# saiakarsh193/GenVox

Hardware: NVIDIA B200
Metric: Tacotron2 train mel-frames/s (higher is better)
Workload: dtype bf16

## Files before the change

genvox_b200/_native.py:

```python
import ctypes as C
import os

from . import build as _build

_P = C.c_void_p


class GvxDims(C.Structure):
    _fields_ = [("n_mels", C.c_int32), ("enc_dim", C.c_int32), ("att_rnn_dim", C.c_int32), ("dec_rnn_dim", C.c_int32),
                ("prenet_dim", C.c_int32), ("att_dim", C.c_int32), ("loc_filters", C.c_int32), ("loc_kernel", C.c_int32),
                ("p_att_dropout", C.c_float), ("p_dec_dropout", C.c_float), ("precision", C.c_int32)]


PARAM_FIELDS = [
    ("prenet_w0", "prenet.layers.0.linear_layer.weight"),
    ("prenet_w1", "prenet.layers.1.linear_layer.weight"),
    ("att_w_ih", "attention_rnn.weight_ih"),
    ("att_w_hh", "attention_rnn.weight_hh"),
    ("att_b_ih", "attention_rnn.bias_ih"),
    ("att_b_hh", "attention_rnn.bias_hh"),
    ("query_w", "attention_layer.query_layer.linear_layer.weight"),
    ("memory_w", "attention_layer.memory_layer.linear_layer.weight"),
    ("v_w", "attention_layer.v.linear_layer.weight"),
    ("loc_conv_w", "attention_layer.location_layer.location_conv.conv.weight"),
# ... 39 lines not shown
    "gvx_dec_packed_bytes": (C.c_size_t, [C.POINTER(GvxDims)]),
    "gvx_dec_pack_weights": (C.c_int, [C.POINTER(GvxDims), C.POINTER(GvxWeights), _P, _P]),
    "gvx_dec_stash_bytes": (C.c_size_t, [C.POINTER(GvxDims), C.c_int, C.c_int, C.c_int]),
    "gvx_dec_bwd_workspace_bytes": (C.c_size_t, [C.POINTER(GvxDims), C.c_int, C.c_int, C.c_int]),
    "gvx_dec_infer_workspace_bytes": (C.c_size_t, [C.POINTER(GvxDims), C.c_int, C.c_int, C.c_int]),
    "gvx_dec_train_fwd": (C.c_int, [C.POINTER(GvxDims), C.POINTER(GvxWeights), _P, _P, _P, _P, C.c_int, C.c_int, C.c_int,
                                    C.c_uint64, C.c_int, C.c_int, _P, _P, _P, _P, _P]),
    "gvx_dec_train_bwd": (C.c_int, [C.POINTER(GvxDims), C.POINTER(GvxWeights), _P, _P, _P, C.c_int, C.c_int, C.c_int,
                                    C.c_uint64, C.c_int, C.c_int, _P, _P, _P, _P, _P, C.POINTER(GvxGrads), _P, _P]),
    "gvx_dec_infer": (C.c_int, [C.POINTER(GvxDims), C.POINTER(GvxWeights), _P, _P, _P, C.c_int, C.c_int, C.c_int,
                                C.c_float, C.c_int, C.c_uint64, C.c_int, C.c_int, _P, _P, _P, _P, C.POINTER(C.c_int), _P, _P]),
    "gvx_dec_infer_continuous_workspace_bytes": (C.c_size_t, [C.POINTER(GvxDims), C.c_int, C.c_int, C.c_int]),
    "gvx_dec_infer_continuous": (C.c_int, [C.POINTER(GvxDims), C.POINTER(GvxWeights), _P, _P, _P, C.c_int, C.c_int, C.c_int,
                                           C.c_int, _P, C.c_float, C.c_int, C.c_uint64, C.c_int, _P, _P, _P, _P,
                                           C.POINTER(C.c_longlong), _P, _P]),
    "gvx_dec_session_workspace_bytes": (C.c_size_t, [C.POINTER(GvxDims), C.c_int, C.c_int, C.c_int]),
    "gvx_dec_session_init": (C.c_int, [C.POINTER(GvxDims), C.POINTER(GvxSession), _P, _P]),
    "gvx_dec_session_submit": (C.c_int, [C.POINTER(GvxDims), C.POINTER(GvxWeights), _P, C.POINTER(GvxSession), _P, _P, _P,
                                         C.c_int, _P, _P]),
    "gvx_dec_session_step": (C.c_int, [C.POINTER(GvxDims), C.POINTER(GvxWeights), _P, C.POINTER(GvxSession), C.c_int,
                                       _P, _P, _P, _P, _P, C.POINTER(C.c_int), _P, _P]),
    "gvx_test_tc_gemm": (C.c_int, [_P, _P, C.c_int, C.c_int, C.c_int, C.c_int, _P, _P]),
    "gvx_test_nt_gemm": (C.c_int, [_P, _P, C.c_int, C.c_int, C.c_int, C.c_int, _P, _P]),
    "gvx_bench_nt_gemm": (C.c_int, [C.c_int, C.c_int, C.c_int, C.c_int, C.POINTER(C.c_float)]),
    "gvx_test_lstm_chain": (C.c_int, [_P, _P, C.c_int, C.c_int, C.c_int, C.c_float, C.c_uint64, C.c_int, _P, _P, _P, _P, _P, _P]),
    "gvx_debug_timeline": (C.c_int, [_P]),
    "gvx_debug_option": (C.c_int, [C.c_char_p, C.c_int]),
    "gvx_prenet_fwd": (C.c_int, [C.POINTER(GvxDims), C.POINTER(GvxWeights), _P, C.c_int, C.c_int, C.c_uint64, C.c_int,
                                 C.c_int, _P, _P, _P]),
    "gvx_lstm_step": (C.c_int, [C.POINTER(GvxDims), _P, C.c_int, _P, _P, _P, C.c_int, C.c_uint64, C.c_int, C.c_int,
                                C.c_int, _P, _P, _P, _P]),
    "gvx_attention_step": (C.c_int, [C.POINTER(GvxDims), C.POINTER(GvxWeights), _P, _P, _P, _P, _P, C.c_int, C.c_int,
                                     _P, _P, _P, _P, _P, _P]),
}

EXPORTS = sorted(_SIGNATURES)
_lib = None


def library_path():
    return _build.LIB_PATH


def library_is_fresh():
    return _build.is_fresh()


# ... 37 lines not shown
```

genvox_b200/csrc/gvx_bf16_api.cuh:

```cuda
#pragma once
#include <cublas_v2.h>

#include "gvx_attention_c2.cuh"
#include "gvx_bf16.cuh"
#include "gvx_blas.cuh"
#include "gvx_layout.cuh"
#include "gvx_misc.cuh"
#include "gvx_fused_fwd.cuh"
#include "gvx_fused_bwd.cuh"
#include "gvx_nt_gemm.cuh"
#include "gvx_infer_prenet.cuh"
#include "gvx_persist.cuh"

namespace gvx {

typedef __nv_bfloat16 bf16;

inline int round_up(int x, int m) { return (x + m - 1) / m * m; }

struct BfGeom {
    int Kpa, Kpd, Kpq, Kpp, Dp;
    int Ta, Td, Tq, Tp;
    int TaT, TdT, TqT;
    int G4A, G4H;
// ... 884 lines not shown
size_t bwd_total_bf16(const Dims &d, int B, int N, int T) { return BwdBfL(d, B, N, T).total; }
size_t infer_total_bf16(const Dims &d, int B, int N, int steps) { return InferBfL(d, B, N, steps).total; }
size_t stash_seed_off_bf16(const Dims &d, int B, int N, int T) { return StashBfL(d, B, N, T).SEED; }
size_t infer_flags_off_bf16(const Dims &d, int B, int N, int steps) { return InferBfL(d, B, N, steps).FLAGS; }
size_t infer_err_off_bf16(const Dims &d, int B, int N, int steps) { return InferBfL(d, B, N, steps).ERR; }
int check_tc_err_public(int *err_dev, cudaStream_t st, const char *what) { return check_tc_err(err_dev, st, what); }

}

extern "C" int gvx_debug_option(const char *name, int value) {
    if (!strcmp(name, "fused")) gvx::fa_mode() = value;
    else if (!strcmp(name, "persistent")) gvx::pc_mode() = value;
    else { snprintf(gvx::g_err, sizeof(gvx::g_err), "gvx_debug_option: unknown option %s", name); return 1; }
    return 0;
}

extern "C" int gvx_debug_timeline(void *device_buffer) {
    gvx::pc_dbg_buffer() = (long long *)device_buffer;
    return 0;
}

extern "C" int gvx_test_nt_gemm(const float *A, const float *B, int M, int N, int K, int mode, float *C, void *stream) {
    using namespace gvx;
    GVX_CHECK(A && B && C && M > 0 && N > 0 && K > 0 && K % 8 == 0, "bad argument");
    cudaStream_t st = (cudaStream_t)stream;
    bf16 *a = nullptr, *b = nullptr, *at = nullptr, *bt = nullptr;
    int *err = nullptr;
    float *ws = nullptr;
    const size_t ws_floats = (size_t)32 << 20;
    GVX_CUDA(cudaMalloc(&a, (size_t)M * K * 2));
    GVX_CUDA(cudaMalloc(&b, (size_t)N * K * 2));
    GVX_CUDA(cudaMalloc(&err, 64));
    GVX_CUDA(cudaMalloc(&ws, ws_floats * 4));
    GVX_CUDA(cudaMemsetAsync(err, 0, 64, st));
    int rc = 0;
    if (mode == 0) {
        k_to_bf16<<<grid_for((size_t)M * K), 256, 0, st>>>(A, K, (size_t)M, K, a, K);
        k_to_bf16<<<grid_for((size_t)N * K), 256, 0, st>>>(B, K, (size_t)N, K, b, K);
        rc = nt_gemm_bf16(st, M, N, K, a, K, b, K, C, N, err, ws, ws_floats);
    } else {
        GVX_CHECK(M % 8 == 0 && N % 8 == 0, "mode 1 needs M, N multiples of 8");
        k_to_bf16<<<grid_for((size_t)M * K), 256, 0, st>>>(A, M, (size_t)K, M, a, M);
        k_to_bf16<<<grid_for((size_t)N * K), 256, 0, st>>>(B, N, (size_t)K, N, b, N);
        rc = tn_gemm_bf16(st, M, N, K, a, M, b, N, C, N, err, ws, ws_floats);
    }
    if (!rc) rc = check_tc_err(err, st, "nt_gemm");
    else cudaStreamSynchronize(st);
    cudaFree(a); cudaFree(b); cudaFree(at); cudaFree(bt); cudaFree(err); cudaFree(ws);
    return rc;
}

extern "C" int gvx_bench_nt_gemm(int M, int N, int K, int reps, float *ms_out) {
    using namespace gvx;
    bf16 *a = nullptr, *b = nullptr;
    float *c = nullptr, *ws = nullptr;
    int *err = nullptr;
    const size_t ws_floats = (size_t)32 << 20;
    GVX_CUDA(cudaMalloc(&ws, ws_floats * 4));
    GVX_CUDA(cudaMalloc(&a, (size_t)M * K * 2));
    GVX_CUDA(cudaMalloc(&b, (size_t)N * K * 2));
    GVX_CUDA(cudaMalloc(&c, (size_t)M * N * 4));
    GVX_CUDA(cudaMalloc(&err, 64));
    GVX_CUDA(cudaMemset(a, 0, (size_t)M * K * 2));
    GVX_CUDA(cudaMemset(b, 0, (size_t)N * K * 2));
    GVX_CUDA(cudaMemset(err, 0, 64));
    cudaEvent_t e0, e1;
    cudaEventCreate(&e0); cudaEventCreate(&e1);
    int rc = nt_gemm_bf16(0, M, N, K, a, K, b, K, c, N, err, ws, ws_floats);
    cudaEventRecord(e0, 0);
    for (int i = 0; i < reps && !rc; ++i) rc = nt_gemm_bf16(0, M, N, K, a, K, b, K, c, N, err, ws, ws_floats);
    cudaEventRecord(e1, 0);
    cudaEventSynchronize(e1);
    float ms = 0.f;
    cudaEventElapsedTime(&ms, e0, e1);
    *ms_out = ms / (reps > 0 ? reps : 1);
    if (!rc) rc = check_tc_err(err, 0, "nt_gemm bench");
    cudaFree(a); cudaFree(b); cudaFree(c); cudaFree(err); cudaFree(ws);
    cudaEventDestroy(e0); cudaEventDestroy(e1);
    return rc;
}

__global__ void k_bf16_rows_to_f32(const __nv_bfloat16 *__restrict__ x, size_t n, float *__restrict__ y) {
    for (size_t i = (size_t)blockIdx.x * blockDim.x + threadIdx.x; i < n; i += (size_t)gridDim.x * blockDim.x) y[i] = __bfloat162float(x[i]);
}

extern "C" int gvx_test_lstm_chain(const float *w_hh, const float *pre, int B, int T, int H, float p_drop, uint64_t seed,
                                   int training, float *h_out, float *c_out, float *gates_out, const float *dh_ext,
                                   float *dgates_out, void *stream) {
    using namespace gvx;
    GVX_CHECK(w_hh && pre && h_out && c_out && gates_out && B > 0 && T > 0, "bad argument");
    GVX_CHECK(pc_supported(H, B), "persistent chain: unsupported shape (need H % 64 == 0, H/8 <= SM count, B <= 64)");
    cudaStream_t st = (cudaStream_t)stream;
    bf16 *wimg = nullptr, *wimgT = nullptr, *himg = nullptr, *hrm = nullptr, *gimg = nullptr, *dgrm = nullptr;
// ... 44 lines not shown
```

genvox_b200/csrc/gvx_nt_gemm.cuh:

```cuda
#pragma once
#include <cuda.h>
#include <cuda_bf16.h>

#include "gvx_tc.cuh"

namespace gvx {

constexpr int NG_BM = 128, NG_BN = 256, NG_BK = 64;
constexpr int NG_STAGES = 4;
constexpr int NG_STAGE_BYTES = (NG_BM + NG_BN) * NG_BK * 2;
constexpr int NG_THREADS = 192;

struct NgShared {
    uint64_t full[NG_STAGES], empty[NG_STAGES], tfull[2], tempty[2];
    uint32_t tmem_slot;
};
constexpr size_t NG_SMEM = (size_t)NG_STAGES * NG_STAGE_BYTES + sizeof(NgShared) + 1024;

__device__ __forceinline__ void tma_load_2d(void *smem_dst, const CUtensorMap *tm, int c0, int c1, uint64_t *bar) {
    asm volatile("cp.async.bulk.tensor.2d.shared::cluster.global.tile.mbarrier::complete_tx::bytes [%0], [%1, {%2, %3}], [%4];" ::"r"(
                     smem_u32(smem_dst)),
                 "l"(reinterpret_cast<uint64_t>(tm)), "r"(c0), "r"(c1), "r"(smem_u32(bar))
                 : "memory");
}
__device__ __forceinline__ void tmem_ld32(uint32_t taddr, float *v) {
    uint32_t r[32];
    asm volatile(
        "tcgen05.ld.sync.aligned.32x32b.x32.b32 "
        "{%0, %1, %2, %3, %4, %5, %6, %7, %8, %9, %10, %11, %12, %13, %14, %15, %16, %17, %18, %19, %20, %21, %22, %23, %24, %25, %26, "
        "%27, %28, %29, %30, %31}, [%32];"
        : "=r"(r[0]), "=r"(r[1]), "=r"(r[2]), "=r"(r[3]), "=r"(r[4]), "=r"(r[5]), "=r"(r[6]), "=r"(r[7]), "=r"(r[8]), "=r"(r[9]),
          "=r"(r[10]), "=r"(r[11]), "=r"(r[12]), "=r"(r[13]), "=r"(r[14]), "=r"(r[15]), "=r"(r[16]), "=r"(r[17]), "=r"(r[18]),
          "=r"(r[19]), "=r"(r[20]), "=r"(r[21]), "=r"(r[22]), "=r"(r[23]), "=r"(r[24]), "=r"(r[25]), "=r"(r[26]), "=r"(r[27]),
          "=r"(r[28]), "=r"(r[29]), "=r"(r[30]), "=r"(r[31])
        : "r"(taddr));
    asm volatile("tcgen05.wait::ld.sync.aligned;" ::: "memory");
#pragma unroll
    for (int i = 0; i < 32; ++i) v[i] = __uint_as_float(r[i]);
}
__device__ __forceinline__ void mbar_arrive_local(uint64_t *bar) {
    asm volatile("mbarrier.arrive.shared::cta.b64 _, [%0];" ::"r"(smem_u32(bar)) : "memory");
}

struct NgArgs {
    float *C;
    int M, N, K, ldc, tiles_m, tiles_n;
    int splits;
    float *P;
    int *err;
};

template <bool MN>
__global__ void __launch_bounds__(NG_THREADS, 1) k_nt_gemm(const __grid_constant__ CUtensorMap tmA, const __grid_constant__ CUtensorMap tmB,
                                                           const NgArgs a) {
    extern __shared__ uint8_t smem_raw[];
    uint8_t *smem = smem_raw + ((1024u - (smem_u32(smem_raw) & 1023u)) & 1023u);
    NgShared *sh = (NgShared *)(smem + (size_t)NG_STAGES * NG_STAGE_BYTES);
    const int warp = threadIdx.x >> 5, lane = threadIdx.x & 31;
    const int ntiles = a.tiles_m * a.tiles_n * a.splits, nkb_all = (a.K + NG_BK - 1) / NG_BK;
    auto item_of = [&](int item, int &tm, int &tn, int &kb0, int &kb1, int &sp) {
        const int t = item / a.splits;
        sp = item - t * a.splits;
        tm = t / a.tiles_n;
        tn = t - tm * a.tiles_n;
        kb0 = (int)((long long)nkb_all * sp / a.splits);
        kb1 = (int)((long long)nkb_all * (sp + 1) / a.splits);
    };

    if (threadIdx.x == 0) {
        for (int s = 0; s < NG_STAGES; ++s) { mbar_init(sh->full + s, 1); mbar_init(sh->empty + s, 1); }
        for (int k = 0; k < 2; ++k) { mbar_init(sh->tfull + k, 1); mbar_init(sh->tempty + k, 4); }
        asm volatile("fence.mbarrier_init.release.cluster;" ::: "memory");
        asm volatile("fence.proxy.async.shared::cta;" ::: "memory");
    }
    if (warp == 0) {
        asm volatile("tcgen05.alloc.cta_group::1.sync.aligned.shared::cta.b32 [%0], %1;" ::"r"(smem_u32(&sh->tmem_slot)), "n"(512) : "memory");
        asm volatile("tcgen05.relinquish_alloc_permit.cta_group::1.sync.aligned;" ::: "memory");
    }
    tc_fence_before();
    __syncthreads();
    tc_fence_after();
    const uint32_t tmem_base = sh->tmem_slot;

    if (warp == 0) {
        if (elect_one()) {
            int s = 0;
            uint32_t ph = 0;
            for (int tile = blockIdx.x; tile < ntiles; tile += gridDim.x) {
                int tm, tn, kb0, kb1, sp;
                item_of(tile, tm, tn, kb0, kb1, sp);
                for (int kb = kb0; kb < kb1; ++kb) {
                    if (!mbar_wait(sh->empty + s, ph ^ 1u, a.err, 71)) return;
                    uint8_t *dst = smem + (size_t)s * NG_STAGE_BYTES;
                    mbar_expect_tx(sh->full + s, NG_STAGE_BYTES);
                    if (MN) {
#pragma unroll
                        for (int q = 0; q < NG_BM / 64; ++q) tma_load_2d(dst + q * 8192, &tmA, tm * NG_BM + 64 * q, kb * NG_BK, sh->full + s);
#pragma unroll
                        for (int q = 0; q < NG_BN / 64; ++q)
                            tma_load_2d(dst + NG_BM * NG_BK * 2 + q * 8192, &tmB, tn * NG_BN + 64 * q, kb * NG_BK, sh->full + s);
                    } else {
                        tma_load_2d(dst, &tmA, kb * NG_BK, tm * NG_BM, sh->full + s);
                        tma_load_2d(dst + NG_BM * NG_BK * 2, &tmB, kb * NG_BK, tn * NG_BN, sh->full + s);
                    }
                    if (++s == NG_STAGES) { s = 0; ph ^= 1u; }
                }
            }
        }
    } else if (warp == 1) {
        if (elect_one()) {
            constexpr uint32_t idesc = umma_idesc_bf16(NG_BM, NG_BN) | (MN ? (1u << 15) | (1u << 16) : 0u);
            constexpr int kstep = MN ? (2048 >> 4) : 2;
            const uint64_t ad0 = MN ? umma_desc_sw128_mn(smem_u32(smem)) : umma_desc_sw128(smem_u32(smem));
            int s = 0, it = 0;
            uint32_t ph = 0;
            for (int tile = blockIdx.x; tile < ntiles; tile += gridDim.x, ++it) {
                const int acc = it & 1;
                if (!mbar_wait(sh->tempty + acc, (uint32_t)((it >> 1) & 1) ^ 1u, a.err, 72)) return;
                tc_fence_after();
                const uint32_t tacc = tmem_base + (uint32_t)(acc * NG_BN);
                int tm, tn, kb0, kb1, sp;
                item_of(tile, tm, tn, kb0, kb1, sp);
                for (int kb = kb0; kb < kb1; ++kb) {
                    if (!mbar_wait(sh->full + s, ph, a.err, 73)) return;
                    tc_fence_after();
                    const uint64_t ad = ad0 + (uint64_t)(s * (NG_STAGE_BYTES >> 4)), bd = ad + (uint64_t)((NG_BM * NG_BK * 2) >> 4);
#pragma unroll
                    for (int j = 0; j < NG_BK / 16; ++j) umma_bf16(tacc, ad + kstep * j, bd + kstep * j, idesc, (kb > kb0 || j > 0) ? 1u : 0u);
                    umma_commit(sh->empty + s);
                    if (++s == NG_STAGES) { s = 0; ph ^= 1u; }
                }
                umma_commit(sh->tfull + acc);
            }
        }
    } else {
        const int q = warp & 3;
        int it = 0;
        for (int tile = blockIdx.x; tile < ntiles; tile += gridDim.x, ++it) {
            const int acc = it & 1;
            int tm, tn, kb0, kb1, sp;
            item_of(tile, tm, tn, kb0, kb1, sp);
            if (!mbar_wait(sh->tfull + acc, (uint32_t)((it >> 1) & 1), a.err, 74)) return;
            tc_fence_after();
            const int m = tm * NG_BM + 32 * q + lane;
            const int ldc = a.splits > 1 ? a.N : a.ldc;
            float *crow = (a.splits > 1 ? a.P + (size_t)sp * a.M * a.N : a.C) + (size_t)m * ldc + tn * NG_BN;
#pragma unroll 1
            for (int c0 = 0; c0 < NG_BN; c0 += 32) {
                float v[32];
                tmem_ld32(tmem_base + ((uint32_t)(32 * q) << 16) + (uint32_t)(acc * NG_BN + c0), v);
                if (m < a.M) {
                    const int nrem = a.N - (tn * NG_BN + c0);
                    if (nrem >= 32 && (ldc & 3) == 0) {
#pragma unroll
                        for (int i = 0; i < 32; i += 4) *reinterpret_cast<float4 *>(crow + c0 + i) = make_float4(v[i], v[i + 1], v[i + 2], v[i + 3]);
                    } else {
#pragma unroll
                        for (int i = 0; i < 32; ++i)
                            if (i < nrem) crow[c0 + i] = v[i];
                    }
                }
            }
            tc_fence_before();
            __syncwarp();
            if (lane == 0) mbar_arrive_local(sh->tempty + acc);
        }
    }
    __syncthreads();
    if (warp == 0) {
        asm volatile("tcgen05.dealloc.cta_group::1.sync.aligned.b32 %0, %1;" ::"r"(tmem_base), "n"(512) : "memory");
    }
}

typedef CUresult (*PFN_encodeTiled)(CUtensorMap *, CUtensorMapDataType, cuuint32_t, void *, const cuuint64_t *, const cuuint64_t *,
                                    const cuuint32_t *, const cuuint32_t *, CUtensorMapInterleave, CUtensorMapSwizzle,
                                    CUtensorMapL2promotion, CUtensorMapFloatOOBfill);
inline PFN_encodeTiled ng_encode_fn() {
    static PFN_encodeTiled fn = nullptr;
    if (!fn) {
        void *p = nullptr;
        cudaDriverEntryPointQueryResult q;
        if (cudaGetDriverEntryPoint("cuTensorMapEncodeTiled", &p, cudaEnableDefault, &q) == cudaSuccess && q == cudaDriverEntryPointSuccess)
            fn = (PFN_encodeTiled)p;
    }
    return fn;
}
inline int ng_tensor_map_mn(CUtensorMap *tm, const __nv_bfloat16 *base, int K, int MNsize, int ld) {
    PFN_encodeTiled fn = ng_encode_fn();
    GVX_CHECK(fn != nullptr, "cuTensorMapEncodeTiled is not available from this driver");
    GVX_CHECK(((uintptr_t)base & 15) == 0 && ld % 8 == 0, "tn_gemm: operands must be 16-byte aligned with a row stride that is a multiple of 8");
    const cuuint64_t dims[2] = {(cuuint64_t)MNsize, (cuuint64_t)K};
    const cuuint64_t strides[1] = {(cuuint64_t)ld * 2};
    const cuuint32_t box[2] = {64u, (cuuint32_t)NG_BK};
// ... 12 lines not shown
    GVX_CHECK(((uintptr_t)base & 15) == 0 && ld % 8 == 0, "nt_gemm: operands must be 16-byte aligned with a row stride that is a multiple of 8");
    const cuuint64_t dims[2] = {(cuuint64_t)K, (cuuint64_t)rows};
    const cuuint64_t strides[1] = {(cuuint64_t)ld * 2};
    const cuuint32_t box[2] = {(cuuint32_t)NG_BK, (cuuint32_t)box_rows};
    const cuuint32_t estr[2] = {1, 1};
    const CUresult r = fn(tm, CU_TENSOR_MAP_DATA_TYPE_BFLOAT16, 2, (void *)base, dims, strides, box, estr, CU_TENSOR_MAP_INTERLEAVE_NONE,
                          CU_TENSOR_MAP_SWIZZLE_128B, CU_TENSOR_MAP_L2_PROMOTION_L2_256B, CU_TENSOR_MAP_FLOAT_OOB_FILL_NONE);
    if (r != CUDA_SUCCESS) {
        snprintf(g_err, sizeof(g_err), "cuTensorMapEncodeTiled failed: %d (rows %d, K %d, ld %d)", (int)r, rows, K, ld);
        return 1;
    }
    return 0;
}

__global__ void __launch_bounds__(256) k_ng_reduce_splits(const float *__restrict__ P, int splits, int M, int N, float *__restrict__ C, int ldc) {
    const size_t total = (size_t)M * N;
    for (size_t i = (size_t)blockIdx.x * blockDim.x + threadIdx.x; i < total; i += (size_t)gridDim.x * blockDim.x) {
        float s = 0.f;
        for (int k = 0; k < splits; ++k) s += P[(size_t)k * total + i];
        C[(i / N) * ldc + (i % N)] = s;
    }
}

inline int ng_gemm_bf16(bool mn, cudaStream_t st, int M, int N, int K, const __nv_bfloat16 *A, int lda, const __nv_bfloat16 *B, int ldb,
                       float *C, int ldc, int *err, float *ws, size_t ws_floats) {
    GVX_CHECK(M > 0 && N > 0 && K > 0 && (mn || K % 8 == 0), "nt_gemm: bad shape");
    CUtensorMap tmA, tmB;
    if (mn) {
        GVX_TRY(ng_tensor_map_mn(&tmA, A, K, M, lda));
        GVX_TRY(ng_tensor_map_mn(&tmB, B, K, N, ldb));
    } else {
        GVX_TRY(ng_tensor_map(&tmA, A, M, K, lda, NG_BM));
        GVX_TRY(ng_tensor_map(&tmB, B, N, K, ldb, NG_BN));
    }
    NgArgs a;
    a.C = C; a.M = M; a.N = N; a.K = K; a.ldc = ldc; a.err = err;
    a.tiles_m = (M + NG_BM - 1) / NG_BM; a.tiles_n = (N + NG_BN - 1) / NG_BN;
    a.splits = 1; a.P = nullptr;
    static int sms = 0;
    if (!sms) {
        int dev = 0;
        cudaGetDevice(&dev);
        cudaDeviceGetAttribute(&sms, cudaDevAttrMultiProcessorCount, dev);
        GVX_CUDA(cudaFuncSetAttribute(k_nt_gemm<false>, cudaFuncAttributeMaxDynamicSharedMemorySize, (int)NG_SMEM));
        GVX_CUDA(cudaFuncSetAttribute(k_nt_gemm<true>, cudaFuncAttributeMaxDynamicSharedMemorySize, (int)NG_SMEM));
    }
    int ntiles = a.tiles_m * a.tiles_n;
    const int nkb = (K + NG_BK - 1) / NG_BK;
    if (ws && nkb >= 128) {
        auto eff = [&](int sp) {
            const int items = ntiles * sp, waves = (items + sms - 1) / sms;
            return (double)items / ((double)waves * sms);
        };
        int best = 1;
        double best_eff = eff(1);
        for (int sp = 2; sp <= 64 && nkb / sp >= 64; ++sp) {
            if ((size_t)sp * M * N > ws_floats) break;
            const double e = eff(sp);
            if (e > best_eff + 0.03) { best = sp; best_eff = e; }
        }
        if (best > 1) { a.splits = best; a.P = ws; ntiles *= best; }
    }
    if (mn) k_nt_gemm<true><<<ntiles < sms ? ntiles : sms, NG_THREADS, NG_SMEM, st>>>(tmA, tmB, a);
    else k_nt_gemm<false><<<ntiles < sms ? ntiles : sms, NG_THREADS, NG_SMEM, st>>>(tmA, tmB, a);
    GVX_LAUNCHED(1);
    GVX_CUDA(cudaGetLastError());
    if (a.splits > 1) {
        const size_t total = (size_t)M * N;
        k_ng_reduce_splits<<<(unsigned)((total + 255) / 256 < 1184 ? (total + 255) / 256 : 1184), 256, 0, st>>>(ws, a.splits, M, N, C, ldc);
        GVX_LAUNCHED(1);
        GVX_CUDA(cudaGetLastError());
    }
    return 0;
}

inline int nt_gemm_bf16(cudaStream_t st, int M, int N, int K, const __nv_bfloat16 *A, int lda, const __nv_bfloat16 *B, int ldb, float *C,
                        int ldc, int *err, float *ws = nullptr, size_t ws_floats = 0) {
    return ng_gemm_bf16(false, st, M, N, K, A, lda, B, ldb, C, ldc, err, ws, ws_floats);
}
inline int tn_gemm_bf16(cudaStream_t st, int M, int N, int K, const __nv_bfloat16 *At, int lda, const __nv_bfloat16 *Bt, int ldb, float *C,
                        int ldc, int *err, float *ws = nullptr, size_t ws_floats = 0) {
    return ng_gemm_bf16(true, st, M, N, K, At, lda, Bt, ldb, C, ldc, err, ws, ws_floats);
}

}
```

include/genvox_b200.h:

```cpp
#ifndef GENVOX_B200_H
#define GENVOX_B200_H

#include <stddef.h>
#include <stdint.h>

#ifdef __cplusplus
extern "C" {
#endif

#define GVX_ABI_VERSION 1
#define GVX_STOP_POLL 16

typedef struct gvx_dims {
    int32_t n_mels;
    int32_t enc_dim;
    int32_t att_rnn_dim;
    int32_t dec_rnn_dim;
    int32_t prenet_dim;
    int32_t att_dim;
    int32_t loc_filters;
    int32_t loc_kernel;
    float p_att_dropout;
    float p_dec_dropout;
    int32_t precision;
// ... 87 lines not shown
    uint64_t seed;
    long long steps_run;
    long long submitted;
    long long admitted;
    long long finished;
    int32_t active;
    int32_t parity;
    int32_t ready;
} gvx_session;

size_t gvx_dec_session_workspace_bytes(const gvx_dims *d, int N, int slots, int capacity);
int gvx_dec_session_init(const gvx_dims *d, gvx_session *s, void *workspace, void *stream);
int gvx_dec_session_submit(const gvx_dims *d, const gvx_weights *w, const void *packed, gvx_session *s,
                           const float *memory, const int64_t *lengths, const int32_t *frame_caps, int k,
                           void *workspace, void *stream);
int gvx_dec_session_step(const gvx_dims *d, const gvx_weights *w, const void *packed, gvx_session *s, int max_steps_this_call,
                         float *frames, float *align, int32_t *utt, int32_t *frame, int8_t *last, int *steps_run,
                         void *workspace, void *stream);


int gvx_test_tc_gemm(const float *W, const float *X, int B, int Mtot, int K, int KS, float *out, void *stream);

int gvx_test_nt_gemm(const float *A, const float *B, int M, int N, int K, int mode, float *C, void *stream);
int gvx_bench_nt_gemm(int M, int N, int K, int reps, float *ms_out);

int gvx_test_lstm_chain(const float *w_hh, const float *pre, int B, int T, int H, float p_drop, uint64_t seed,
                        int training, float *h_out, float *c_out, float *gates_out, const float *dh_ext,
                        float *dgates_out, void *stream);

int gvx_debug_timeline(void *device_buffer);

int gvx_debug_option(const char *name, int value);

int gvx_prenet_fwd(const gvx_dims *d, const gvx_weights *w, const float *frames, int F, int B,
                   uint64_t seed, int t0, int row_offset, float *tmp, float *out, void *stream);

int gvx_lstm_step(const gvx_dims *d, const void *packed, int which, const float *x, const float *h,
                  const float *c, int B, uint64_t seed, int t, int training, int row_offset,
                  float *h_out, float *c_out, float *gates_out, void *stream);

int gvx_attention_step(const gvx_dims *d, const gvx_weights *w, const void *packed, const float *h_att, const float *memory,
                       const float *processed_memory, const int64_t *mem_lengths, int B, int N,
                       float *w_prev, float *w_cum, float *q_tmp, float *ctx_out, float *align_out,
                       void *stream);

#ifdef __cplusplus
}
// ... 3 lines not shown
```

profiles/nt_gemm_bench.py:

```python
import ctypes as C
import os
import sys

import torch

sys.path.insert(0, os.path.dirname(os.path.dirname(os.path.abspath(__file__))))
from genvox_b200 import _native

lib = _native.load()
TB = 51200
shapes = [("dW dec-LSTM      (4096 x 2560, K = frames)", 4096, 2560, TB), ("dW att-LSTM      (4096 x 1792, K = frames)", 4096, 1792, TB),
          ("dW query         (128 x 1024, K = frames)", 128, 1024, TB), ("dW projections   (81 x 1536, K = frames)", 88, 1536, TB),
          ("dec gates input  (frames x 4096, K = 1536)", TB, 4096, 1536), ("att gates prenet (frames x 4096, K = 256)", TB, 4096, 256),
          ("d [h_att|ctx]    (frames x 1536, K = 4096)", TB, 1536, 4096), ("d prenet_out     (frames x 256, K = 4096)", TB, 256, 4096),
          ("projections      (frames x 81, K = 1536)", TB, 88, 1536)]
dev = torch.device("cuda:0")
for name, M, N, K in shapes:
    ms = C.c_float(0)
    _native.check(lib.gvx_bench_nt_gemm(M, N, K, 5, C.byref(ms)), "gvx_bench_nt_gemm")
    a = torch.zeros(M, K, dtype=torch.bfloat16, device=dev)
    b = torch.zeros(N, K, dtype=torch.bfloat16, device=dev)
    for _ in range(2):
        c = a @ b.t()
    e0, e1 = torch.cuda.Event(enable_timing=True), torch.cuda.Event(enable_timing=True)
    e0.record()
    for _ in range(5):
        c = a @ b.t()
    e1.record()
    torch.cuda.synchronize()
    tms = e0.elapsed_time(e1) / 5
    fl = 2.0 * M * N * K
    print(f"{name:46s} own {ms.value:7.3f} ms = {fl / ms.value / 1e9:7.1f} TFLOP/s   cuBLAS(bf16 out) {tms:7.3f} ms = {fl / tms / 1e9:7.1f} TFLOP/s")
    del a, b, c
```

Before: 1.399 million.

## Use 2-CTA cluster tcgen05 MMA for bulk NT/TN GEMMs with deeper SMEM ring

Adds a cta_group::2 variant of the persistent tcgen05 GEMM. Two CTAs in a cluster share a 256x256 MMA tile, and each loads half of the B operand. Stage count is now derived from a fixed 192 KB ring, so the pair path gets more pipeline stages. This is meant to halve per-CTA B traffic and SMEM footprint and improve tensor-core utilization for the large dW and projection GEMMs, and the paired path is the default. It adds cluster launch, multicast commit and remote mbarrier complexity, plus a drain loop before teardown.

After: 1.409 million (median of 6 runs). About the same (+0.7%).

```diff
diff --git a/genvox_b200/_native.py b/genvox_b200/_native.py
--- a/genvox_b200/_native.py
+++ b/genvox_b200/_native.py
@@ -85,7 +85,7 @@
                                        _P, _P, _P, _P, _P, C.POINTER(C.c_int), _P, _P]),
     "gvx_test_tc_gemm": (C.c_int, [_P, _P, C.c_int, C.c_int, C.c_int, C.c_int, _P, _P]),
     "gvx_test_nt_gemm": (C.c_int, [_P, _P, C.c_int, C.c_int, C.c_int, C.c_int, _P, _P]),
-    "gvx_bench_nt_gemm": (C.c_int, [C.c_int, C.c_int, C.c_int, C.c_int, C.POINTER(C.c_float)]),
+    "gvx_bench_nt_gemm": (C.c_int, [C.c_int, C.c_int, C.c_int, C.c_int, C.c_int, C.POINTER(C.c_float)]),
     "gvx_test_lstm_chain": (C.c_int, [_P, _P, C.c_int, C.c_int, C.c_int, C.c_float, C.c_uint64, C.c_int, _P, _P, _P, _P, _P, _P]),
     "gvx_debug_timeline": (C.c_int, [_P]),
     "gvx_debug_option": (C.c_int, [C.c_char_p, C.c_int]),
diff --git a/genvox_b200/csrc/gvx_bf16_api.cuh b/genvox_b200/csrc/gvx_bf16_api.cuh
--- a/genvox_b200/csrc/gvx_bf16_api.cuh
+++ b/genvox_b200/csrc/gvx_bf16_api.cuh
@@ -930,9 +930,10 @@
 
 extern "C" int gvx_test_nt_gemm(const float *A, const float *B, int M, int N, int K, int mode, float *C, void *stream) {
     using namespace gvx;
-    GVX_CHECK(A && B && C && M > 0 && N > 0 && K > 0 && K % 8 == 0, "bad argument");
+    GVX_CHECK(A && B && C && M > 0 && N > 0 && K > 0 && K % 8 == 0 && mode >= 0 && mode <= 3, "bad argument");
     cudaStream_t st = (cudaStream_t)stream;
-    bf16 *a = nullptr, *b = nullptr, *at = nullptr, *bt = nullptr;
+    const bool mn = (mode & 1) != 0, pair = mode < 2;
+    bf16 *a = nullptr, *b = nullptr;
     int *err = nullptr;
     float *ws = nullptr;
     const size_t ws_floats = (size_t)32 << 20;
@@ -942,24 +943,28 @@
     GVX_CUDA(cudaMalloc(&ws, ws_floats * 4));
     GVX_CUDA(cudaMemsetAsync(err, 0, 64, st));
     int rc = 0;
-    if (mode == 0) {
+    if (!mn) {
         k_to_bf16<<<grid_for((size_t)M * K), 256, 0, st>>>(A, K, (size_t)M, K, a, K);
         k_to_bf16<<<grid_for((size_t)N * K), 256, 0, st>>>(B, K, (size_t)N, K, b, K);
-        rc = nt_gemm_bf16(st, M, N, K, a, K, b, K, C, N, err, ws, ws_floats);
+        rc = ng_gemm_bf16(false, st, M, N, K, a, K, b, K, C, N, err, ws, ws_floats, pair);
     } else {
-        GVX_CHECK(M % 8 == 0 && N % 8 == 0, "mode 1 needs M, N multiples of 8");
+        GVX_CHECK(M % 8 == 0 && N % 8 == 0, "modes 1 and 3 need M, N multiples of 8");
         k_to_bf16<<<grid_for((size_t)M * K), 256, 0, st>>>(A, M, (size_t)K, M, a, M);
         k_to_bf16<<<grid_for((size_t)N * K), 256, 0, st>>>(B, N, (size_t)K, N, b, N);
-        rc = tn_gemm_bf16(st, M, N, K, a, M, b, N, C, N, err, ws, ws_floats);
+        rc = ng_gemm_bf16(true, st, M, N, K, a, M, b, N, C, N, err, ws, ws_floats, pair);
     }
     if (!rc) rc = check_tc_err(err, st, "nt_gemm");
     else cudaStreamSynchronize(st);
-    cudaFree(a); cudaFree(b); cudaFree(at); cudaFree(bt); cudaFree(err); cudaFree(ws);
+    cudaFree(a); cudaFree(b); cudaFree(err); cudaFree(ws);
     return rc;
 }
 
-extern "C" int gvx_bench_nt_gemm(int M, int N, int K, int reps, float *ms_out) {
+extern "C" int gvx_bench_nt_gemm(int M, int N, int K, int mode, int reps, float *ms_out) {
     using namespace gvx;
+    GVX_CHECK(M > 0 && N > 0 && K > 0 && K % 8 == 0 && mode >= 0 && mode <= 5 && ms_out, "bad argument");
+    const bool mn = (mode & 1) != 0;
+    const int engine = mode >> 1;
+    GVX_CHECK(!mn || (M % 8 == 0 && N % 8 == 0), "the TN form needs M, N multiples of 8");
     bf16 *a = nullptr, *b = nullptr;
     float *c = nullptr, *ws = nullptr;
     int *err = nullptr;
@@ -972,11 +977,16 @@
     GVX_CUDA(cudaMemset(a, 0, (size_t)M * K * 2));
     GVX_CUDA(cudaMemset(b, 0, (size_t)N * K * 2));
     GVX_CUDA(cudaMemset(err, 0, 64));
+    auto run = [&]() -> int {
+        if (engine == 2) return mn ? gemm_tn_bf16(0, M, N, K, a, M, b, N, c, N) : gemm_nt_bf16(0, M, N, K, a, K, b, K, c, N);
+        return mn ? ng_gemm_bf16(true, 0, M, N, K, a, M, b, N, c, N, err, ws, ws_floats, engine == 0)
+                  : ng_gemm_bf16(false, 0, M, N, K, a, K, b, K, c, N, err, ws, ws_floats, engine == 0);
+    };
     cudaEvent_t e0, e1;
     cudaEventCreate(&e0); cudaEventCreate(&e1);
-    int rc = nt_gemm_bf16(0, M, N, K, a, K, b, K, c, N, err, ws, ws_floats);
+    int rc = run();
     cudaEventRecord(e0, 0);
-    for (int i = 0; i < reps && !rc; ++i) rc = nt_gemm_bf16(0, M, N, K, a, K, b, K, c, N, err, ws, ws_floats);
+    for (int i = 0; i < reps && !rc; ++i) rc = run();
     cudaEventRecord(e1, 0);
     cudaEventSynchronize(e1);
     float ms = 0.f;
diff --git a/genvox_b200/csrc/gvx_nt_gemm.cuh b/genvox_b200/csrc/gvx_nt_gemm.cuh
--- a/genvox_b200/csrc/gvx_nt_gemm.cuh
+++ b/genvox_b200/csrc/gvx_nt_gemm.cuh
@@ -7,21 +7,70 @@
 namespace gvx {
 
 constexpr int NG_BM = 128, NG_BN = 256, NG_BK = 64;
-constexpr int NG_STAGES = 4;
-constexpr int NG_STAGE_BYTES = (NG_BM + NG_BN) * NG_BK * 2;
+constexpr int NG_RING_BYTES = 192 * 1024;
 constexpr int NG_THREADS = 192;
+constexpr int NG_MAX_STAGES = 8;
 
 struct NgShared {
-    uint64_t full[NG_STAGES], empty[NG_STAGES], tfull[2], tempty[2];
+    uint64_t full[NG_MAX_STAGES], empty[NG_MAX_STAGES], tfull[2], tempty[2];
     uint32_t tmem_slot;
 };
-constexpr size_t NG_SMEM = (size_t)NG_STAGES * NG_STAGE_BYTES + sizeof(NgShared) + 1024;
-
-__device__ __forceinline__ void tma_load_2d(void *smem_dst, const CUtensorMap *tm, int c0, int c1, uint64_t *bar) {
-    asm volatile("cp.async.bulk.tensor.2d.shared::cluster.global.tile.mbarrier::complete_tx::bytes [%0], [%1, {%2, %3}], [%4];" ::"r"(
-                     smem_u32(smem_dst)),
-                 "l"(reinterpret_cast<uint64_t>(tm)), "r"(c0), "r"(c1), "r"(smem_u32(bar))
-                 : "memory");
+template <int CG>
+struct NgCfg {
+    static constexpr int BN_CTA = NG_BN / CG;
+    static constexpr int A_BYTES = NG_BM * NG_BK * 2;
+    static constexpr int STAGE_BYTES = (NG_BM + BN_CTA) * NG_BK * 2;
+    static constexpr int STAGES = NG_RING_BYTES / STAGE_BYTES;
+    static constexpr size_t SMEM = (size_t)NG_RING_BYTES + sizeof(NgShared) + 1024;
+    static_assert(STAGES <= NG_MAX_STAGES && STAGES * STAGE_BYTES == NG_RING_BYTES, "ring layout");
+};
+
+template <int CG>
+__device__ __forceinline__ void ng_tma_load(void *smem_dst, const CUtensorMap *tm, int c0, int c1, uint32_t bar) {
+    if constexpr (CG == 2)
+        asm volatile("cp.async.bulk.tensor.2d.cta_group::2.shared::cluster.global.mbarrier::complete_tx::bytes [%0], [%1, {%2, %3}], [%4];" ::"r"(
+                         smem_u32(smem_dst)),
+                     "l"(reinterpret_cast<uint64_t>(tm)), "r"(c0), "r"(c1), "r"(bar)
+                     : "memory");
+    else
+        asm volatile("cp.async.bulk.tensor.2d.shared::cluster.global.tile.mbarrier::complete_tx::bytes [%0], [%1, {%2, %3}], [%4];" ::"r"(
+                         smem_u32(smem_dst)),
+                     "l"(reinterpret_cast<uint64_t>(tm)), "r"(c0), "r"(c1), "r"(bar)
+                     : "memory");
+}
+template <int CG>
+__device__ __forceinline__ void ng_umma(uint32_t tmem_d, uint64_t adesc, uint64_t bdesc, uint32_t idesc, uint32_t accumulate) {
+    if constexpr (CG == 2)
+        asm volatile(
+            "{\n\t.reg .pred p;\n\t"
+            "setp.ne.b32 p, %4, 0;\n\t"
+            "tcgen05.mma.cta_group::2.kind::f16 [%0], %1, %2, %3, p;\n\t}" ::"r"(tmem_d),
+            "l"(adesc), "l"(bdesc), "r"(idesc), "r"(accumulate)
+            : "memory");
+    else
+        umma_bf16(tmem_d, adesc, bdesc, idesc, accumulate);
+}
+template <int CG>
+__device__ __forceinline__ void ng_commit(uint64_t *bar) {
+    if constexpr (CG == 2)
+        asm volatile("tcgen05.commit.cta_group::2.mbarrier::arrive::one.shared::cluster.multicast::cluster.b64 [%0], %1;" ::"r"(smem_u32(bar)),
+                     "h"((uint16_t)3)
+                     : "memory");
+    else
+        umma_commit(bar);
+}
+__device__ __forceinline__ uint32_t ng_cta_rank() {
+    uint32_t r;
+    asm volatile("mov.u32 %0, %%cluster_ctarank;" : "=r"(r));
+    return r;
+}
+__device__ __forceinline__ uint32_t ng_mapa(uint32_t saddr, uint32_t rank) {
+    uint32_t r;
+    asm volatile("mapa.shared::cluster.u32 %0, %1, %2;" : "=r"(r) : "r"(saddr), "r"(rank));
+    return r;
+}
+__device__ __forceinline__ void ng_cluster_sync() {
+    asm volatile("barrier.cluster.arrive.release;\n\tbarrier.cluster.wait.acquire;" ::: "memory");
 }
 __device__ __forceinline__ void tmem_ld32(uint32_t taddr, float *v) {
     uint32_t r[32];
@@ -38,9 +87,6 @@
 #pragma unroll
     for (int i = 0; i < 32; ++i) v[i] = __uint_as_float(r[i]);
 }
-__device__ __forceinline__ void mbar_arrive_local(uint64_t *bar) {
-    asm volatile("mbarrier.arrive.shared::cta.b64 _, [%0];" ::"r"(smem_u32(bar)) : "memory");
-}
 
 struct NgArgs {
     float *C;
@@ -50,13 +96,17 @@
     int *err;
 };
 
-template <bool MN>
+template <bool MN, int CG>
 __global__ void __launch_bounds__(NG_THREADS, 1) k_nt_gemm(const __grid_constant__ CUtensorMap tmA, const __grid_constant__ CUtensorMap tmB,
                                                            const NgArgs a) {
+    using Cfg = NgCfg<CG>;
+    constexpr int STAGES = Cfg::STAGES, SB = Cfg::STAGE_BYTES;
     extern __shared__ uint8_t smem_raw[];
     uint8_t *smem = smem_raw + ((1024u - (smem_u32(smem_raw) & 1023u)) & 1023u);
-    NgShared *sh = (NgShared *)(smem + (size_t)NG_STAGES * NG_STAGE_BYTES);
+    NgShared *sh = (NgShared *)(smem + NG_RING_BYTES);
     const int warp = threadIdx.x >> 5, lane = threadIdx.x & 31;
+    const uint32_t rank = CG == 2 ? ng_cta_rank() : 0u;
+    const int unit = (int)blockIdx.x / CG, nunits = (int)gridDim.x / CG;
     const int ntiles = a.tiles_m * a.tiles_n * a.splits, nkb_all = (a.K + NG_BK - 1) / NG_BK;
     auto item_of = [&](int item, int &tm, int &tn, int &kb0, int &kb1, int &sp) {
         const int t = item / a.splits;
@@ -68,81 +118,97 @@
     };
 
     if (threadIdx.x == 0) {
-        for (int s = 0; s < NG_STAGES; ++s) { mbar_init(sh->full + s, 1); mbar_init(sh->empty + s, 1); }
-        for (int k = 0; k < 2; ++k) { mbar_init(sh->tfull + k, 1); mbar_init(sh->tempty + k, 4); }
+        for (int s = 0; s < STAGES; ++s) { mbar_init(sh->full + s, 1); mbar_init(sh->empty + s, 1); }
+        for (int k = 0; k < 2; ++k) { mbar_init(sh->tfull + k, 1); mbar_init(sh->tempty + k, 4 * CG); }
         asm volatile("fence.mbarrier_init.release.cluster;" ::: "memory");
         asm volatile("fence.proxy.async.shared::cta;" ::: "memory");
     }
     if (warp == 0) {
-        asm volatile("tcgen05.alloc.cta_group::1.sync.aligned.shared::cta.b32 [%0], %1;" ::"r"(smem_u32(&sh->tmem_slot)), "n"(512) : "memory");
-        asm volatile("tcgen05.relinquish_alloc_permit.cta_group::1.sync.aligned;" ::: "memory");
+        if constexpr (CG == 2) {
+            asm volatile("tcgen05.alloc.cta_group::2.sync.aligned.shared::cta.b32 [%0], %1;" ::"r"(smem_u32(&sh->tmem_slot)), "n"(512) : "memory");
+            asm volatile("tcgen05.relinquish_alloc_permit.cta_group::2.sync.aligned;" ::: "memory");
+        } else {
+            asm volatile("tcgen05.alloc.cta_group::1.sync.aligned.shared::cta.b32 [%0], %1;" ::"r"(smem_u32(&sh->tmem_slot)), "n"(512) : "memory");
+            asm volatile("tcgen05.relinquish_alloc_permit.cta_group::1.sync.aligned;" ::: "memory");
+        }
     }
     tc_fence_before();
     __syncthreads();
+    if constexpr (CG == 2) ng_cluster_sync();
     tc_fence_after();
     const uint32_t tmem_base = sh->tmem_slot;
 
     if (warp == 0) {
         if (elect_one()) {
+            const uint32_t full0 = CG == 2 ? ng_mapa(smem_u32(sh->full), 0u) : smem_u32(sh->full);
             int s = 0;
             uint32_t ph = 0;
-            for (int tile = blockIdx.x; tile < ntiles; tile += gridDim.x) {
+            bool ok = true;
+            for (int tile = unit; ok && tile < ntiles; tile += nunits) {
                 int tm, tn, kb0, kb1, sp;
                 item_of(tile, tm, tn, kb0, kb1, sp);
+                const int arow = tm * (NG_BM * CG) + (int)rank * NG_BM, brow = tn * NG_BN + (int)rank * Cfg::BN_CTA;
                 for (int kb = kb0; kb < kb1; ++kb) {
-                    if (!mbar_wait(sh->empty + s, ph ^ 1u, a.err, 71)) return;
-                    uint8_t *dst = smem + (size_t)s * NG_STAGE_BYTES;
-                    mbar_expect_tx(sh->full + s, NG_STAGE_BYTES);
+                    if (!mbar_wait(sh->empty + s, ph ^ 1u, a.err, 71)) { ok = false; break; }
+                    uint8_t *dst = smem + (size_t)s * SB;
+                    const uint32_t fb = full0 + (uint32_t)(s * 8);
+                    if (rank == 0) mbar_expect_tx(sh->full + s, (uint32_t)(CG * SB));
                     if (MN) {
 #pragma unroll
-                        for (int q = 0; q < NG_BM / 64; ++q) tma_load_2d(dst + q * 8192, &tmA, tm * NG_BM + 64 * q, kb * NG_BK, sh->full + s);
-#pragma unroll
-                        for (int q = 0; q < NG_BN / 64; ++q)
-                            tma_load_2d(dst + NG_BM * NG_BK * 2 + q * 8192, &tmB, tn * NG_BN + 64 * q, kb * NG_BK, sh->full + s);
+                        for (int q = 0; q < NG_BM / 64; ++q) ng_tma_load<CG>(dst + q * 8192, &tmA, arow + 64 * q, kb * NG_BK, fb);
+#pragma unroll
+                        for (int q = 0; q < Cfg::BN_CTA / 64; ++q)
+                            ng_tma_load<CG>(dst + Cfg::A_BYTES + q * 8192, &tmB, brow + 64 * q, kb * NG_BK, fb);
                     } else {
-                        tma_load_2d(dst, &tmA, kb * NG_BK, tm * NG_BM, sh->full + s);
-                        tma_load_2d(dst + NG_BM * NG_BK * 2, &tmB, kb * NG_BK, tn * NG_BN, sh->full + s);
+                        ng_tma_load<CG>(dst, &tmA, kb * NG_BK, arow, fb);
+                        ng_tma_load<CG>(dst + Cfg::A_BYTES, &tmB, kb * NG_BK, brow, fb);
                     }
-                    if (++s == NG_STAGES) { s = 0; ph ^= 1u; }
+                    if (++s == STAGES) { s = 0; ph ^= 1u; }
                 }
             }
+            for (int i = 0; ok && i < STAGES; ++i) {
+                if (!mbar_wait(sh->empty + s, ph ^ 1u, a.err, 75)) ok = false;
+                if (++s == STAGES) { s = 0; ph ^= 1u; }
+            }
         }
     } else if (warp == 1) {
-        if (elect_one()) {
-            constexpr uint32_t idesc = umma_idesc_bf16(NG_BM, NG_BN) | (MN ? (1u << 15) | (1u << 16) : 0u);
+        if (rank == 0 && elect_one()) {
+            constexpr uint32_t idesc = umma_idesc_bf16(NG_BM * CG, NG_BN) | (MN ? (1u << 15) | (1u << 16) : 0u);
             constexpr int kstep = MN ? (2048 >> 4) : 2;
             const uint64_t ad0 = MN ? umma_desc_sw128_mn(smem_u32(smem)) : umma_desc_sw128(smem_u32(smem));
             int s = 0, it = 0;
             uint32_t ph = 0;
-            for (int tile = blockIdx.x; tile < ntiles; tile += gridDim.x, ++it) {
+            bool ok = true;
+            for (int tile = unit; ok && tile < ntiles; tile += nunits, ++it) {
                 const int acc = it & 1;
-                if (!mbar_wait(sh->tempty + acc, (uint32_t)((it >> 1) & 1) ^ 1u, a.err, 72)) return;
+                if (!mbar_wait(sh->tempty + acc, (uint32_t)((it >> 1) & 1) ^ 1u, a.err, 72)) break;
                 tc_fence_after();
                 const uint32_t tacc = tmem_base + (uint32_t)(acc * NG_BN);
                 int tm, tn, kb0, kb1, sp;
                 item_of(tile, tm, tn, kb0, kb1, sp);
                 for (int kb = kb0; kb < kb1; ++kb) {
-                    if (!mbar_wait(sh->full + s, ph, a.err, 73)) return;
+                    if (!mbar_wait(sh->full + s, ph, a.err, 73)) { ok = false; break; }
                     tc_fence_after();
-                    const uint64_t ad = ad0 + (uint64_t)(s * (NG_STAGE_BYTES >> 4)), bd = ad + (uint64_t)((NG_BM * NG_BK * 2) >> 4);
-#pragma unroll
-                    for (int j = 0; j < NG_BK / 16; ++j) umma_bf16(tacc, ad + kstep * j, bd + kstep * j, idesc, (kb > kb0 || j > 0) ? 1u : 0u);
-                    umma_commit(sh->empty + s);
-                    if (++s == NG_STAGES) { s = 0; ph ^= 1u; }
+                    const uint64_t ad = ad0 + (uint64_t)(s * (SB >> 4)), bd = ad + (uint64_t)(Cfg::A_BYTES >> 4);
+#pragma unroll
+                    for (int j = 0; j < NG_BK / 16; ++j) ng_umma<CG>(tacc, ad + kstep * j, bd + kstep * j, idesc, (kb > kb0 || j > 0) ? 1u : 0u);
+                    ng_commit<CG>(sh->empty + s);
+                    if (++s == STAGES) { s = 0; ph ^= 1u; }
                 }
-                umma_commit(sh->tfull + acc);
+                if (ok) ng_commit<CG>(sh->tfull + acc);
             }
         }
     } else {
         const int q = warp & 3;
+        const uint32_t tempty0 = CG == 2 ? ng_mapa(smem_u32(sh->tempty), 0u) : smem_u32(sh->tempty);
         int it = 0;
-        for (int tile = blockIdx.x; tile < ntiles; tile += gridDim.x, ++it) {
+        for (int tile = unit; tile < ntiles; tile += nunits, ++it) {
             const int acc = it & 1;
             int tm, tn, kb0, kb1, sp;
             item_of(tile, tm, tn, kb0, kb1, sp);
-            if (!mbar_wait(sh->tfull + acc, (uint32_t)((it >> 1) & 1), a.err, 74)) return;
+            if (!mbar_wait(sh->tfull + acc, (uint32_t)((it >> 1) & 1), a.err, 74)) break;
             tc_fence_after();
-            const int m = tm * NG_BM + 32 * q + lane;
+            const int m = tm * (NG_BM * CG) + (int)rank * NG_BM + 32 * q + lane;
             const int ldc = a.splits > 1 ? a.N : a.ldc;
             float *crow = (a.splits > 1 ? a.P + (size_t)sp * a.M * a.N : a.C) + (size_t)m * ldc + tn * NG_BN;
 #pragma unroll 1
@@ -163,12 +229,20 @@
             }
             tc_fence_before();
             __syncwarp();
-            if (lane == 0) mbar_arrive_local(sh->tempty + acc);
-        }
-    }
+            if (lane == 0) {
+                const uint32_t bar = tempty0 + (uint32_t)(acc * 8);
+                if constexpr (CG == 2) asm volatile("mbarrier.arrive.release.cluster.shared::cluster.b64 _, [%0];" ::"r"(bar) : "memory");
+                else asm volatile("mbarrier.arrive.shared::cta.b64 _, [%0];" ::"r"(bar) : "memory");
+            }
+        }
+    }
+    tc_fence_before();
     __syncthreads();
+    if constexpr (CG == 2) ng_cluster_sync();
+    tc_fence_after();
     if (warp == 0) {
-        asm volatile("tcgen05.dealloc.cta_group::1.sync.aligned.b32 %0, %1;" ::"r"(tmem_base), "n"(512) : "memory");
+        if constexpr (CG == 2) asm volatile("tcgen05.dealloc.cta_group::2.sync.aligned.b32 %0, %1;" ::"r"(tmem_base), "n"(512) : "memory");
+        else asm volatile("tcgen05.dealloc.cta_group::1.sync.aligned.b32 %0, %1;" ::"r"(tmem_base), "n"(512) : "memory");
     }
 }
 
@@ -227,8 +301,84 @@
     }
 }
 
+template <bool MN, int CG>
+inline int ng_units(int *out) {
+    static int units = 0;
+    if (!units) {
+        auto kern = k_nt_gemm<MN, CG>;
+        GVX_CUDA(cudaFuncSetAttribute(kern, cudaFuncAttributeMaxDynamicSharedMemorySize, (int)NgCfg<CG>::SMEM));
+        int dev = 0, sms = 0;
+        GVX_CUDA(cudaGetDevice(&dev));
+        GVX_CUDA(cudaDeviceGetAttribute(&sms, cudaDevAttrMultiProcessorCount, dev));
+        units = sms;
+        if (CG > 1) {
+            cudaLaunchConfig_t cfg;
+            memset(&cfg, 0, sizeof(cfg));
+            cfg.gridDim = dim3(CG * (sms / CG));
+            cfg.blockDim = dim3(NG_THREADS);
+            cfg.dynamicSmemBytes = NgCfg<CG>::SMEM;
+            cudaLaunchAttribute attr[1];
+            attr[0].id = cudaLaunchAttributeClusterDimension;
+            attr[0].val.clusterDim.x = CG; attr[0].val.clusterDim.y = 1; attr[0].val.clusterDim.z = 1;
+            cfg.attrs = attr;
+            cfg.numAttrs = 1;
+            GVX_CUDA(cudaOccupancyMaxActiveClusters(&units, kern, &cfg));
+            GVX_CHECK(units > 0, "nt_gemm: no CTA pair of the paired GEMM fits on this device");
+        }
+    }
+    *out = units;
+    return 0;
+}
+
+template <bool MN, int CG>
+inline int ng_launch(cudaStream_t st, int M, int N, int K, const CUtensorMap &tmA, const CUtensorMap &tmB, float *C, int ldc, int *err,
+                     float *ws, size_t ws_floats) {
+    NgArgs a;
+    a.C = C; a.M = M; a.N = N; a.K = K; a.ldc = ldc; a.err = err;
+    a.tiles_m = (M + NG_BM * CG - 1) / (NG_BM * CG); a.tiles_n = (N + NG_BN - 1) / NG_BN;
+    a.splits = 1; a.P = nullptr;
+    int units = 0;
+    GVX_TRY((ng_units<MN, CG>(&units)));
+    int ntiles = a.tiles_m * a.tiles_n;
+    const int nkb = (K + NG_BK - 1) / NG_BK;
+    if (ws && nkb >= 128) {
+        auto eff = [&](int sp) {
+            const int items = ntiles * sp, waves = (items + units - 1) / units;
+            return (double)items / ((double)waves * units);
+        };
+        int best = 1;
+        double best_eff = eff(1);
+        for (int sp = 2; sp <= 64 && nkb / sp >= 64; ++sp) {
+            if ((size_t)sp * M * N > ws_floats) break;
+            const double e = eff(sp);
+            if (e > best_eff + 0.03) { best = sp; best_eff = e; }
+        }
+        if (best > 1) { a.splits = best; a.P = ws; ntiles *= best; }
+    }
+    cudaLaunchConfig_t cfg;
+    memset(&cfg, 0, sizeof(cfg));
+    cfg.gridDim = dim3(CG * (ntiles < units ? ntiles : units));
+    cfg.blockDim = dim3(NG_THREADS);
+    cfg.dynamicSmemBytes = NgCfg<CG>::SMEM;
+    cfg.stream = st;
+    cudaLaunchAttribute attr[1];
+    attr[0].id = cudaLaunchAttributeClusterDimension;
+    attr[0].val.clusterDim.x = CG; attr[0].val.clusterDim.y = 1; attr[0].val.clusterDim.z = 1;
+    cfg.attrs = attr;
+    cfg.numAttrs = 1;
+    GVX_CUDA(cudaLaunchKernelEx(&cfg, k_nt_gemm<MN, CG>, tmA, tmB, a));
+    GVX_LAUNCHED(1);
+    if (a.splits > 1) {
+        const size_t total = (size_t)M * N;
+        k_ng_reduce_splits<<<(unsigned)((total + 255) / 256 < 1184 ? (total + 255) / 256 : 1184), 256, 0, st>>>(ws, a.splits, M, N, C, ldc);
+        GVX_LAUNCHED(1);
+        GVX_CUDA(cudaGetLastError());
+    }
+    return 0;
+}
+
 inline int ng_gemm_bf16(bool mn, cudaStream_t st, int M, int N, int K, const __nv_bfloat16 *A, int lda, const __nv_bfloat16 *B, int ldb,
-                       float *C, int ldc, int *err, float *ws, size_t ws_floats) {
+                       float *C, int ldc, int *err, float *ws, size_t ws_floats, bool pair = true) {
     GVX_CHECK(M > 0 && N > 0 && K > 0 && (mn || K % 8 == 0), "nt_gemm: bad shape");
     CUtensorMap tmA, tmB;
     if (mn) {
@@ -236,47 +386,12 @@
         GVX_TRY(ng_tensor_map_mn(&tmB, B, K, N, ldb));
     } else {
         GVX_TRY(ng_tensor_map(&tmA, A, M, K, lda, NG_BM));
-        GVX_TRY(ng_tensor_map(&tmB, B, N, K, ldb, NG_BN));
-    }
-    NgArgs a;
-    a.C = C; a.M = M; a.N = N; a.K = K; a.ldc = ldc; a.err = err;
-    a.tiles_m = (M + NG_BM - 1) / NG_BM; a.tiles_n = (N + NG_BN - 1) / NG_BN;
-    a.splits = 1; a.P = nullptr;
-    static int sms = 0;
-    if (!sms) {
-        int dev = 0;
-        cudaGetDevice(&dev);
-        cudaDeviceGetAttribute(&sms, cudaDevAttrMultiProcessorCount, dev);
-        GVX_CUDA(cudaFuncSetAttribute(k_nt_gemm<false>, cudaFuncAttributeMaxDynamicSharedMemorySize, (int)NG_SMEM));
-        GVX_CUDA(cudaFuncSetAttribute(k_nt_gemm<true>, cudaFuncAttributeMaxDynamicSharedMemorySize, (int)NG_SMEM));
-    }
-    int ntiles = a.tiles_m * a.tiles_n;
-    const int nkb = (K + NG_BK - 1) / NG_BK;
-    if (ws && nkb >= 128) {
-        auto eff = [&](int sp) {
-            const int items = ntiles * sp, waves = (items + sms - 1) / sms;
-            return (double)items / ((double)waves * sms);
-        };
-        int best = 1;
-        double best_eff = eff(1);
-        for (int sp = 2; sp <= 64 && nkb / sp >= 64; ++sp) {
-            if ((size_t)sp * M * N > ws_floats) break;
-            const double e = eff(sp);
-            if (e > best_eff + 0.03) { best = sp; best_eff = e; }
-        }
-        if (best > 1) { a.splits = best; a.P = ws; ntiles *= best; }
-    }
-    if (mn) k_nt_gemm<true><<<ntiles < sms ? ntiles : sms, NG_THREADS, NG_SMEM, st>>>(tmA, tmB, a);
-    else k_nt_gemm<false><<<ntiles < sms ? ntiles : sms, NG_THREADS, NG_SMEM, st>>>(tmA, tmB, a);
-    GVX_LAUNCHED(1);
-    GVX_CUDA(cudaGetLastError());
-    if (a.splits > 1) {
-        const size_t total = (size_t)M * N;
-        k_ng_reduce_splits<<<(unsigned)((total + 255) / 256 < 1184 ? (total + 255) / 256 : 1184), 256, 0, st>>>(ws, a.splits, M, N, C, ldc);
-        GVX_LAUNCHED(1);
-        GVX_CUDA(cudaGetLastError());
-    }
-    return 0;
+        GVX_TRY(ng_tensor_map(&tmB, B, N, K, ldb, pair ? NgCfg<2>::BN_CTA : NgCfg<1>::BN_CTA));
+    }
+    if (pair) return mn ? ng_launch<true, 2>(st, M, N, K, tmA, tmB, C, ldc, err, ws, ws_floats)
+                        : ng_launch<false, 2>(st, M, N, K, tmA, tmB, C, ldc, err, ws, ws_floats);
+    return mn ? ng_launch<true, 1>(st, M, N, K, tmA, tmB, C, ldc, err, ws, ws_floats)
+              : ng_launch<false, 1>(st, M, N, K, tmA, tmB, C, ldc, err, ws, ws_floats);
 }
 
 inline int nt_gemm_bf16(cudaStream_t st, int M, int N, int K, const __nv_bfloat16 *A, int lda, const __nv_bfloat16 *B, int ldb, float *C,
diff --git a/include/genvox_b200.h b/include/genvox_b200.h
--- a/include/genvox_b200.h
+++ b/include/genvox_b200.h
@@ -133,7 +133,7 @@
 int gvx_test_tc_gemm(const float *W, const float *X, int B, int Mtot, int K, int KS, float *out, void *stream);
 
 int gvx_test_nt_gemm(const float *A, const float *B, int M, int N, int K, int mode, float *C, void *stream);
-int gvx_bench_nt_gemm(int M, int N, int K, int reps, float *ms_out);
+int gvx_bench_nt_gemm(int M, int N, int K, int mode, int reps, float *ms_out);
 
 int gvx_test_lstm_chain(const float *w_hh, const float *pre, int B, int T, int H, float p_drop, uint64_t seed,
                         int training, float *h_out, float *c_out, float *gates_out, const float *dh_ext,
diff --git a/profiles/nt_gemm_bench.py b/profiles/nt_gemm_bench.py
--- a/profiles/nt_gemm_bench.py
+++ b/profiles/nt_gemm_bench.py
@@ -1,5 +1,8 @@
+import argparse
 import ctypes as C
+import json
 import os
+import subprocess
 import sys
 
 import torch
@@ -7,28 +10,64 @@
 sys.path.insert(0, os.path.dirname(os.path.dirname(os.path.abspath(__file__))))
 from genvox_b200 import _native
 
-lib = _native.load()
 TB = 51200
-shapes = [("dW dec-LSTM      (4096 x 2560, K = frames)", 4096, 2560, TB), ("dW att-LSTM      (4096 x 1792, K = frames)", 4096, 1792, TB),
-          ("dW query         (128 x 1024, K = frames)", 128, 1024, TB), ("dW projections   (81 x 1536, K = frames)", 88, 1536, TB),
-          ("dec gates input  (frames x 4096, K = 1536)", TB, 4096, 1536), ("att gates prenet (frames x 4096, K = 256)", TB, 4096, 256),
-          ("d [h_att|ctx]    (frames x 1536, K = 4096)", TB, 1536, 4096), ("d prenet_out     (frames x 256, K = 4096)", TB, 256, 4096),
-          ("projections      (frames x 81, K = 1536)", TB, 88, 1536)]
-dev = torch.device("cuda:0")
-for name, M, N, K in shapes:
-    ms = C.c_float(0)
-    _native.check(lib.gvx_bench_nt_gemm(M, N, K, 5, C.byref(ms)), "gvx_bench_nt_gemm")
-    a = torch.zeros(M, K, dtype=torch.bfloat16, device=dev)
-    b = torch.zeros(N, K, dtype=torch.bfloat16, device=dev)
-    for _ in range(2):
-        c = a @ b.t()
-    e0, e1 = torch.cuda.Event(enable_timing=True), torch.cuda.Event(enable_timing=True)
-    e0.record()
-    for _ in range(5):
-        c = a @ b.t()
-    e1.record()
-    torch.cuda.synchronize()
-    tms = e0.elapsed_time(e1) / 5
-    fl = 2.0 * M * N * K
-    print(f"{name:46s} own {ms.value:7.3f} ms = {fl / ms.value / 1e9:7.1f} TFLOP/s   cuBLAS(bf16 out) {tms:7.3f} ms = {fl / tms / 1e9:7.1f} TFLOP/s")
-    del a, b, c
+SHAPES = [
+    ("fwd att-LSTM gates, prenet part", "NT", TB, 4096, 256),
+    ("fwd dec-LSTM gates, input part", "NT", TB, 4096, 1536),
+    ("fwd mel / gate projections", "NT", TB, 81, 1536),
+    ("bwd d [h_att | ctx]", "NT", TB, 1536, 4096),
+    ("bwd d prenet_out", "NT", TB, 256, 4096),
+    ("bwd d W_proj", "TN", 88, 1536, TB),
+    ("bwd d W_dec", "TN", 4096, 2560, TB),
+    ("bwd d W_att", "TN", 4096, 1792, TB),
+    ("bwd d W_q", "TN", 128, 1024, TB),
+]
+ENGINES = [("paired", 0), ("single", 1), ("cuBLAS", 2)]
+
+
+def card():
+    info = {"device": torch.cuda.get_device_name(0)}
+    try:
+        out = subprocess.run(["nvidia-smi", "-i", "0", "--query-gpu=power.limit,clocks.max.sm,clocks.sm", "--format=csv,noheader"],
+                             capture_output=True, text=True, timeout=30).stdout.strip()
+        info["power_limit, max SM clock, SM clock"] = out
+    except (OSError, subprocess.SubprocessError) as e:
+        info["power_limit, max SM clock, SM clock"] = f"unavailable ({e})"
+    return info
+
+
+def main():
+    ap = argparse.ArgumentParser()
+    ap.add_argument("--rounds", type=int, default=3)
+    ap.add_argument("--reps", type=int, default=10)
+    ap.add_argument("--json", default=None)
+    args = ap.parse_args()
+    lib = _native.load()
+    info = card()
+    print(json.dumps(info))
+    rows = []
+    tot = {e: 0.0 for e, _ in ENGINES}
+    for name, form, M, N, K in SHAPES:
+        best = {e: float("inf") for e, _ in ENGINES}
+        for _ in range(args.rounds):
+            for e, code in ENGINES:
+                ms = C.c_float(0)
+                _native.check(lib.gvx_bench_nt_gemm(M, N, K, 2 * code + (form == "TN"), args.reps, C.byref(ms)), "gvx_bench_nt_gemm")
+                best[e] = min(best[e], ms.value)
+        fl = 2.0 * M * N * K
+        row = {"site": name, "form": form, "M": M, "N": N, "K": K, "tflop": fl / 1e12}
+        for e, _ in ENGINES:
+            row[e + "_ms"] = best[e]
+            row[e + "_pflops"] = fl / best[e] / 1e12
+            tot[e] += best[e]
+        rows.append(row)
+        print(f"{name:34s} {form} {M:6d} x {N:5d} x {K:6d}  " +
+              "  ".join(f"{e} {best[e]:7.3f} ms {row[e + '_pflops']:5.2f} PF/s" for e, _ in ENGINES), flush=True)
+    print("sum of the call sites: " + "  ".join(f"{e} {tot[e]:.3f} ms" for e, _ in ENGINES))
+    if args.json:
+        with open(args.json, "w") as fh:
+            json.dump({"card": info, "rows": rows, "sum_ms": tot}, fh, indent=1)
+
+
+if __name__ == "__main__":
+    main()
```
